# JohannesErnst/WeaSAL

Hardware: AMD Instinct MI355X
Metric: points/sec fwd+bwd KPFCNN on DALES spheres; achieved HBM GB/s on KPConv gather (higher is better)
Workload: dtype f32; 1 GPU; DALES_PseudoLabel KP-FCNN, in_radius=10m, 50k pts/sphere, batch=8, fp32, step = GPU pyramid + fwd + loss + bwd + SGD; contrast_loss term included (trainer_PseudoLabel.py:204-208); pyramid of the next batch overlapped on a second stream; parallelism=dp1, dist_world_size=1, allreduce_bytes=0

## Files before the change

### weasal_amd/_lib.py

```python
import ctypes as C
import os

_HERE = os.path.dirname(os.path.abspath(__file__))
LIB_PATH = os.path.join(_HERE, "libweasal_hip.so")

_vp = C.c_void_p
_i32 = C.c_int32
_i64 = C.c_int64
_f32 = C.c_float

SIGNATURES = {
    "ws_last_error": (C.c_char_p, []),
    "ws_version": (C.c_char_p, []),
    "ws_device_count": (C.c_int, []),
    "ws_kpconv_gather_fwd": (C.c_int, [_vp, _i64, _vp, _i64, _vp, _i32, _vp, _i32, _vp, _i32, _vp, _vp,
                                      _f32, _i32, _i32, _vp, _vp, _vp, _vp]),
    "ws_kpconv_gather_bwd_x": (C.c_int, [_vp, _i64, _vp, _i64, _vp, _i32, _vp, _vp, _vp, _i32, _vp, _i32,
                                        _vp, _vp, _f32, _i32, _i32, _vp, _vp, _vp]),
    "ws_kpconv_gather_bwd_geom": (C.c_int, [_vp, _i64, _vp, _i64, _vp, _i32, _vp, _i32, _vp, _vp, _i32,
                                           _vp, _vp, _vp, _f32, _i32, _i32, _vp, _vp, _vp]),
    "ws_transpose_scratch_bytes": (_i64, [_i64, _i32, _i64]),
    "ws_transpose_build": (C.c_int, [_vp, _i64, _i32, _i64, _vp, _vp, _vp, _vp]),
    "ws_max_pool_fwd": (C.c_int, [_vp, _i64, _i32, _vp, _i64, _i32, _vp, _vp, _vp]),
    "ws_max_pool_bwd": (C.c_int, [_vp, _vp, _i64, _i32, _i32, _vp, _vp, _i64, _vp, _vp]),
# ... 122 lines not shown
    "ws_region_mean_fwd": (C.c_int, [_vp, _i64, _i32, _vp, _vp, _i64, _vp, _i64, _vp, _vp]),
    "ws_region_mean_bwd": (C.c_int, [_vp, _i64, _i32, _vp, _vp, _i64, _vp, _i64, _vp, _vp]),
    "ws_sampler_create": (C.c_int, [C.POINTER(_vp)]),
    "ws_sampler_destroy": (None, [_vp]),
    "ws_sampler_add_cloud": (C.c_int, [_vp, _vp, _vp, _i64, _vp, _vp, _i64, _vp]),
    "ws_sampler_state_bytes": (_i64, []),
    "ws_sampler_draw_bytes": (_i64, []),
    "ws_sampler_batch": (C.c_int, [_vp, _vp, _i32, _i32, _i64, C.c_double, _f32, C.c_uint64, C.c_uint64, _i32, _vp, _i32, _i32, _i32,
                                   _vp, _vp, _vp, _vp, _vp, _vp, _vp, _vp, _vp, _i64, _vp, _vp]),
    "ws_softmax_ce_scratch_bytes": (_i64, [_i64]),
    "ws_softmax_ce_fwd": (C.c_int, [_vp, _i64, _i32, _i64, _vp, _vp, _i32, _vp, _vp, _vp, _vp, _vp]),
    "ws_softmax_ce_bwd": (C.c_int, [_vp, _i64, _i32, _i64, _vp, _vp, _i32, _vp, _vp, _vp, _vp, _i64, _vp]),
    "ws_sgd_step": (C.c_int, [_vp, _vp, _vp, _vp, _i32, _f32, _f32, _f32, _f32, _i32, _vp]),
    "ws_kpconv_deform_prepare": (C.c_int, [_vp, _i64, _i32, _vp, _i32, _f32, _i32, _vp, _vp, _vp, _vp, _vp]),
    "ws_kpconv_gather_fwd_ex": (C.c_int, [_vp, _i64, _vp, _i64, _vp, _i32, _vp, _i32, _vp, _i32, _vp, _vp, _f32, _i32, _i32, _vp,
                                         _vp, _vp, _i32, _i32, _vp]),
    "ws_kpconv_deform_prepare_bwd": (C.c_int, [_vp, _vp, _vp, _i64, _i32, _i32, _f32, _i32, _vp, _vp]),
    "ws_kpconv_gather_fwd_def": (C.c_int, [_vp, _i64, _vp, _i64, _vp, _i32, _vp, _i32, _vp, _i32, _f32, _vp, _vp, _vp, _i32, _i32, _vp]),
    "ws_kpconv_gather_bwd_x_def": (C.c_int, [_vp, _i64, _vp, _i64, _i32, _vp, _vp, _vp, _i32, _vp, _i32, _f32, _vp, _vp, _i32, _vp]),
    "ws_kpconv_gather_bwd_x_grid_wide": (C.c_int, [_vp, _i64, _vp, _i32, _i64, _vp, _f32, _vp, _i32, _vp, _i32, _vp, _vp, _f32, _vp,
                                                   _vp, _i32, _vp, _i32, _vp]),
    "ws_kpconv_gather_bwd_geom_def": (C.c_int, [_vp, _i64, _vp, _i64, _vp, _i32, _vp, _i32, _vp, _vp, _i32, _vp, _f32, _vp, _vp,
                                                _i32, _i32, _vp]),
    "ws_kpconv_layer_fwd_fused": (C.c_int, [_vp, _i64, _vp, _i64, _vp, _i32, _vp, _i32, _vp, _i32, _f32, _vp, _vp, _i32, _vp, _i32, _f32,
                                           _vp, _vp]),
    "ws_kpconv_gather_fwd_variant": (C.c_int, [_i32, _i32, _i32, _i32, _i32, _i32, C.c_char_p, _i32]),
    "ws_kpconv_gather_variant": (C.c_int, [_i32, _i64, _i64, _i32, _vp, _vp, _i32, _i32, _i32, _i32, _i32, _i32, _i32, C.c_char_p, _i32]),
    "ws_gemm_xb_variant": (C.c_int, [_vp, _i64, _i32, _i64, _vp, _i64, _i64, _i32, _vp, _vp, _i64, _vp, _i64, _vp, _i64, _vp, _i64,
                                     _vp, _i64, C.c_char_p, _i32]),
    "ws_gemm_xty_variant": (C.c_int, [_vp, _i64, _i32, _i64, _vp, _i32, _i64, _vp, _i64, _vp, _i32, C.c_char_p, _i32]),
    "ws_act_bwd_colsum_variant": (C.c_int, [_vp, _i64, _i32, _i64, _vp, _i64, _vp, _i64, _vp, _vp, C.c_char_p, _i32]),
    "ws_gemm_xbt_bf16_variant": (C.c_int, [_i64, _i32, _i32, _vp, _vp, _i64, _vp, _i64, _i32, C.c_char_p, _i32]),
    "ws_act_bwd_colsum_bf16_variant": (C.c_int, [_i32, _i64, _i32, _vp, _vp, C.c_char_p, _i32]),
    "ws_p2p_regularizer_scratch_bytes": (_i64, [_i64]),
    "ws_p2p_regularizer_fwd": (C.c_int, [_vp, _vp, _vp, _i64, _i32, _f32, _f32, _vp, _vp, _vp]),
    "ws_p2p_regularizer_bwd": (C.c_int, [_vp, _vp, _vp, _i64, _i32, _f32, _f32, _vp, _vp, _vp, _vp]),
    "ws_sphere_attention_fwd": (C.c_int, [_vp, _vp, _vp, _i64, _i32, _i32, _vp, _i32, _vp, _vp, _vp, _vp]),
    "ws_sphere_attention_bwd_scratch_bytes": (_i64, [_i64, _i32]),
    "ws_sphere_attention_bwd": (C.c_int, [_vp, _vp, _vp, _vp, _vp, _vp, _vp, _i64, _i32, _i32, _vp, _i32, _vp, _vp, _vp, _vp, _i64, _vp]),
    "ws_channel_attention_scratch_bytes": (_i64, [_vp, _i32, _i32, _i32]),
    "ws_channel_attention_fwd": (C.c_int, [_vp, _vp, _vp, _i64, _i32, _vp, _i32, _i32, _vp, _vp, _vp, _i64, _vp]),
    "ws_channel_attention_bwd": (C.c_int, [_vp, _vp, _vp, _vp, _vp, _i64, _i32, _vp, _i32, _i32, _vp, _vp, _vp, _vp, _i64, _vp]),
    "ws_timer_reset": (C.c_int, []),
    "ws_timer_count": (C.c_int, []),
    "ws_timer_read": (C.c_int, [_i32, _vp, _vp, _vp, _vp]),
    "ws_timer_read_layer": (C.c_int, [_i32, _vp]),
}

ENV_SWITCHES = (
    ("WEASAL_NB_WIDE_CAPS", "ws_nb_wide_caps"),
    ("WEASAL_CLOSEST_BWD_VEC", "ws_closest_bwd_vec"),
    ("WEASAL_GEMM_STAGED", "ws_gemm_staged"),
    ("WEASAL_GEMM_SHALLOW", "ws_gemm_shallow"),
)

_lib = None


class WeasalHipError(RuntimeError):
    pass


def lib():
    global _lib
    if _lib is None:
        if not os.path.exists(LIB_PATH):
            raise WeasalHipError(
                "%s not found: build it with `python -c 'import __graft_entry__ as g; g.build()'` "
                "or `make -C weasal_amd/csrc` (there is no CPU fallback)" % LIB_PATH)
        handle = C.CDLL(LIB_PATH)
        for name, (res, args) in SIGNATURES.items():
            fn = getattr(handle, name)
            fn.restype = res
            fn.argtypes = args
        for env, sym in ENV_SWITCHES:
            if env in os.environ:
                C.c_int.in_dll(handle, sym).value = int(os.environ[env])
        _lib = handle
    return _lib


def check(rc):
    if rc != 0:
        msg = lib().ws_last_error()
        raise WeasalHipError("libweasal_hip status %d: %s" % (rc, msg.decode() if msg else "?"))


def ptr(t):
    return None if t is None else _vp(t.data_ptr())


_raw_stream = None


def current_stream():
    global _raw_stream
    import torch
    if _raw_stream is None:
        get = getattr(torch._C, "_cuda_getCurrentRawStream", None)
        dev = getattr(torch._C, "_cuda_getDevice", None)
        if get is not None and dev is not None and torch.cuda.is_available():
            torch.cuda.current_stream()
            _raw_stream = lambda: get(dev())
        else:
            _raw_stream = lambda: torch.cuda.current_stream().cuda_stream
    return _vp(_raw_stream())
# ... 1 lines not shown
```

### weasal_amd/csrc/kpconv.hip

```cpp
#include "ws_common.h"
#include <algorithm>
#include "ws_grid.h"
#include "ws_bf16.h"

namespace {

constexpr float WS_SHADOW = 1e6f;

struct GeomParams {
    float extent;
    int influence;
    int aggregation;
    int deformable;
    const void* gate;
    float gate_slope;
    const int64_t* rows;
    int rows_h;
    const float4* kp4;
    const float* rmax;
    int cut;
    int ilv;
    int csplit;
};

template <int K>
__device__ __forceinline__ void kp_influence(float nx, float ny, float nz, const float* __restrict__ kp,
                                             const GeomParams& g, bool live, float (&w)[K], float (&d2)[K])
{
    float best = 3.4e38f;
    int arg = 0;
    bool inrange = false;
    const float e2 = g.extent * g.extent;
#pragma unroll
    for (int k = 0; k < K; ++k) {
        const float dx = nx - kp[3 * k + 0];
        const float dy = ny - kp[3 * k + 1];
        const float dz = nz - kp[3 * k + 2];
        const float d = (dx * dx + dy * dy) + dz * dz;
        d2[k] = d;
        if (d < best) { best = d; arg = k; }
        inrange |= d < e2;
    }
#pragma unroll
    for (int k = 0; k < K; ++k) {
        float v;
        if (g.influence == WS_INFLUENCE_LINEAR) {
            v = fmaxf(1.0f - sqrtf(d2[k]) / g.extent, 0.0f);
        } else if (g.influence == WS_INFLUENCE_CONSTANT) {
            v = 1.0f;
        } else {
            const float sig = g.extent * 0.3f;
            v = expf(-d2[k] / (2.0f * sig * sig + 1e-9f));
        }
        if (g.aggregation == WS_AGGREGATION_CLOSEST && k != arg) v = 0.0f;
// ... 1407 lines not shown
            }
        }
#pragma unroll
        for (int r = 0; r < 4; ++r) {
#pragma unroll
            for (int o = 1; o < 16; o <<= 1) {
                gk[r][0] += __shfl_xor(gk[r][0], o, 64);
                gk[r][1] += __shfl_xor(gk[r][1], o, 64);
                gk[r][2] += __shfl_xor(gk[r][2], o, 64);
                gm[r] += __shfl_xor(gm[r], o, 64);
                const float ob = __shfl_xor(best[r], o, 64);
                const int oc = __shfl_xor(bestcol[r], o, 64);
                const bool take = ob < best[r] || (ob == best[r] && oc < bestcol[r]);
                best[r] = take ? ob : best[r];
                bestcol[r] = take ? oc : bestcol[r];
            }
            const int k = 4 * g + r;
            if (k < K) {
                float gx = gk[r][0], gy = gk[r][1], gz = gk[r][2];
                if (d_min_d2) {
                    const int64_t v = inds[q * h + min(bestcol[r], h - 1)];
                    float mx = WS_SHADOW, my = WS_SHADOW, mz = WS_SHADOW;
                    if (v >= 0 && v < ns) { mx = s_pts[3 * v]; my = s_pts[3 * v + 1]; mz = s_pts[3 * v + 2]; }
                    const float gmin = 2.0f * d_min_d2[q * K + k];
                    gx = fmaf(gmin, kq[r].x - (mx - qx), gx);
                    gy = fmaf(gmin, kq[r].y - (my - qy), gy);
                    gz = fmaf(gmin, kq[r].z - (mz - qz), gz);
                }
                if (j == 0) d_kp4[q * K + k] = make_float4(gx, gy, gz, gm[r]);
            }
        }
    }
}

bool aligned16(const void* p) { return (reinterpret_cast<uintptr_t>(p) & 15u) == 0; }

int check_common(const void* q_pts, int64_t nq, const void* s_pts, int64_t ns, int32_t h, int32_t ci,
                 int32_t k, float extent, int32_t influence, int32_t aggregation)
{
    WS_REQUIRE(nq >= 0 && ns >= 0, "negative point count (nq=%lld ns=%lld)", (long long)nq, (long long)ns);
    WS_REQUIRE(h >= 1 && ci >= 1, "h=%d and ci=%d must be >= 1", h, ci);
    WS_REQUIRE(nq == 0 || q_pts, "q_pts is NULL");
    WS_REQUIRE(ns == 0 || s_pts, "s_pts is NULL");
    WS_REQUIRE(extent > 0.0f, "KP_extent must be > 0");
    WS_REQUIRE(influence >= 0 && influence <= 2, "unknown influence %d", influence);
    WS_REQUIRE(aggregation >= 0 && aggregation <= 1, "unknown aggregation %d", aggregation);
    WS_REQUIRE(ns < (1ll << 31) && nq * (int64_t)k < (1ll << 31), "index range exceeds int32");
    if (k != 15) return ws_fail(WS_ERR_UNSUPPORTED, "num_kernel_points=%d: this build instantiates K=15 only", k);
    return WS_OK;
}

constexpr int GRID_SLAB = 192;

template <int K, int G, int MODE, bool VEC, typename T = float, bool SORT = true>
__global__ __launch_bounds__(256) void kpconv_gather_bwd_x_grid_kernel(
    const float* __restrict__ s_pts, int64_t ns, const CloudGrid* __restrict__ grids, int nb,
    const int32_t* __restrict__ cell_start, const float4* __restrict__ sorted,
    const unsigned long long* __restrict__ key_last, float r2, const T* __restrict__ dwf, int ci,
    const float* __restrict__ kernel_points, const float* __restrict__ deformed_kp, const float* __restrict__ modulations,
    GeomParams g, T* __restrict__ dx, const int32_t* __restrict__ order, int32_t* __restrict__ overflow)
{
    constexpr int CC = 4 * G;
    constexpr int S = 64 / G;
    constexpr int EPL = GRID_SLAB / 64;
    __shared__ uint2 pool_all[4][POOL_ALLOC];
    __shared__ int segs_all[4][K + 1];
    __shared__ float4 slab_all[4][GRID_SLAB + 64];
    const int wave = __builtin_amdgcn_readfirstlane(threadIdx.x >> 6);
    const int lane = threadIdx.x & 63;
    uint2* pool = pool_all[wave];
    int* segs = segs_all[wave];
    float4* slab = slab_all[wave];
    const int j = lane % G;
    const int slot = lane / G;
    const float inv_extent = 1.0f / g.extent;

    float kpr[MODE == 0 ? 3 * K : 1];
    if (MODE == 0) {
#pragma unroll
        for (int t = 0; t < 3 * K; ++t) kpr[t] = kernel_points[t];
    }

    int64_t item0, istep, iend;
    ws_wave_items(ns, order ? g.ilv : 0, wave, item0, istep, iend);
    CloudGrid gr = grids[0];
    for (int64_t item = item0; item < iend; item += istep) {
        const int64_t s = order ? (int64_t)order[item] : item;
        if (s < gr.s_base || s >= gr.s_base + gr.s_len) {
            int b = 0;
            while (b + 1 < nb && s >= grids[b].s_base + grids[b].s_len) ++b;
            gr = grids[b];
        }
        const float sx = s_pts[3 * s + 0], sy = s_pts[3 * s + 1], sz = s_pts[3 * s + 2];
        int cnt = 0;
        auto take = [&](const float4& c, bool active) {
            const float d2 = ref_d2(c.x, c.y, c.z, make_float4(sx, sy, sz, 0.0f));
            const unsigned long long key = ((unsigned long long)__float_as_uint(d2) << 32) | (unsigned)s;
            bool hit = active && d2 < r2;
            hit = hit && key <= key_last[hit ? __float_as_int(c.w) : 0];
            const unsigned long long m = __ballot(hit);
            const int pos = cnt + lane_rank(m);
            slab[(hit && pos < GRID_SLAB) ? pos : GRID_SLAB + lane] = c;
            cnt += __builtin_popcountll(m);
        };
        const bool from_row = g.rows != nullptr && key_last[s] == ~0ull;
        if (from_row) {
            for (int h0 = 0; h0 < g.rows_h; h0 += 64) {
                const int col = h0 + lane;
                const int64_t qi = col < g.rows_h ? g.rows[s * g.rows_h + col] : -1;
                const bool active = qi >= 0 && qi < ns;
                const int64_t qq = active ? qi : 0;
                take(make_float4(s_pts[3 * qq + 0], s_pts[3 * qq + 1], s_pts[3 * qq + 2], __int_as_float((int)qq)), active);
            }
        } else if (gr.s_len > 0) {
            const int cx = cell_coord(sx, gr.lo[0], gr.inv_cell);
            const int cy = cell_coord(sy, gr.lo[1], gr.inv_cell);
            const int cz = cell_coord(sz, gr.lo[2], gr.inv_cell);
            const int x0 = max(cx - 1, 0), x1 = min(cx + 1, gr.nx - 1);
            int rb[9], re[9];
#pragma unroll
            for (int r = 0; r < 9; ++r) {
                const int z = cz + r / 3 - 1, y = cy + r % 3 - 1;
                const bool ok = x0 <= x1 && z >= 0 && z < gr.nz && y >= 0 && y < gr.ny;
                const int row = gr.cell_base + ((ok ? z : 0) * gr.ny + (ok ? y : 0)) * gr.nx;
                rb[r] = ok ? cell_start[row + x0] : 0;
                re[r] = ok ? cell_start[row + x1 + 1] : 0;
            }
            float4 c[9];
#pragma unroll
            for (int r = 0; r < 9; ++r) {
                const int p = rb[r] + lane;
                c[r] = sorted[p < re[r] ? p : 0];
            }
#pragma unroll
            for (int r = 0; r < 9; ++r) {
                take(c[r], rb[r] + lane < re[r]);
                for (int p0 = rb[r] + 64; p0 < re[r]; p0 += 64) {
                    const int p = p0 + lane;
                    float4 cc = make_float4(0.f, 0.f, 0.f, 0.f);
                    if (p < re[r]) cc = sorted[p];
                    take(cc, p < re[r]);
                }
            }
        }
        if (cnt > GRID_SLAB) {
            if (lane == 0) atomicMax(overflow, cnt);
            cnt = GRID_SLAB;
        }
        wave_lds_sync();
        if (SORT) {
            float4 e[EPL];
            int rk[EPL];
#pragma unroll
            for (int u = 0; u < EPL; ++u) {
                e[u] = lane + 64 * u < cnt ? slab[lane + 64 * u] : make_float4(0.f, 0.f, 0.f, __int_as_float(0x7fffffff));
                rk[u] = 0;
            }
            if (cnt <= 64) {
                for (int i = 0; i < cnt; ++i) rk[0] += __float_as_int(slab[i].w) < __float_as_int(e[0].w) ? 1 : 0;
            } else if (cnt <= 128) {
                for (int i = 0; i < cnt; ++i) {
                    const int ki = __float_as_int(slab[i].w);
                    rk[0] += ki < __float_as_int(e[0].w) ? 1 : 0;
                    rk[1] += ki < __float_as_int(e[1].w) ? 1 : 0;
                }
            } else {
                for (int i = 0; i < cnt; ++i) {
                    const int ki = __float_as_int(slab[i].w);
#pragma unroll
                    for (int u = 0; u < EPL; ++u) rk[u] += ki < __float_as_int(e[u].w) ? 1 : 0;
                }
            }
            wave_lds_sync();
#pragma unroll
            for (int u = 0; u < EPL; ++u)
                if (lane + 64 * u < cnt) slab[rk[u]] = e[u];
            wave_lds_sync();
        }
        for (int cc0 = 0; cc0 < ci; cc0 += CC) {
            float4 acc = make_float4(0.f, 0.f, 0.f, 0.f);
            const int ch = cc0 + 4 * j;
            const bool chok = VEC ? (ch + 3 < ci) : (ch < ci);
            const int chl = chok ? ch : 0;
            float4 gq = make_float4(1.f, 1.f, 1.f, 1.f);
            if (g.gate && slot == 0) {
                const T* gy = reinterpret_cast<const T*>(g.gate) + s * ci + ch;
                if (VEC) {
                    if (chok) gq = ld4(gy);
                } else {
                    if (ch + 0 < ci) gq.x = ld1(gy + 0);
                    if (ch + 1 < ci) gq.y = ld1(gy + 1);
                    if (ch + 2 < ci) gq.z = ld1(gy + 2);
                    if (ch + 3 < ci) gq.w = ld1(gy + 3);
                }
            }
            auto flush = [&](int total) {
                wave_lds_sync();
                total = min(total, POOL);
                const int per = (total + S - 1) / S;
                const int lo = slot * per;
                const int hi = chok ? min(lo + per, total) : lo;
                for (int it = 0; it < per; it += 4) {
                    float4 v[4];
                    float w[4];
                    uint2 e[4];
#pragma unroll
                    for (int u = 0; u < 4; ++u) {
                        e[u] = pool[min(lo + it + u, POOL + 7)];
                        keep_unconditional(e[u]);
                    }
#pragma unroll
                    for (int u = 0; u < 4; ++u) {
                        const bool ok = lo + it + u < hi;
                        e[u].x = ok ? e[u].x : 0u;
                        w[u] = ok ? __uint_as_float(e[u].y) : 0.0f;
                        v[u] = load_row_piece<VEC>(dwf, e[u].x, ci, chl);
                    }
#pragma unroll
                    for (int u = 0; u < 4; ++u) {
                        acc.x = fmaf(w[u], v[u].x, acc.x);
                        acc.y = fmaf(w[u], v[u].y, acc.y);
                        acc.z = fmaf(w[u], v[u].z, acc.z);
                        acc.w = fmaf(w[u], v[u].w, acc.w);
                    }
                }
                wave_lds_sync();
            };
            for (int p0 = 0; p0 < cnt; p0 += 64) {
                const int p = p0 + lane;
                const bool real = p < cnt;
                const float4 c = real ? slab[p] : make_float4(0.f, 0.f, 0.f, 0.f);
                const int q = real ? __float_as_int(c.w) : 0;
                const float nx = sx - c.x, ny = sy - c.y, nz = sz - c.z;
                const float* lkp = deformed_kp ? deformed_kp + (int64_t)q * (3 * K) : kernel_points;
                const float* lmod = modulations ? modulations + (int64_t)q * K : nullptr;
                auto kp = [&](int k, int cidx) { return MODE == 0 ? kpr[MODE == 0 ? 3 * k + cidx : 0] : lkp[3 * k + cidx]; };
                auto nomin = [&](int, float) {};
                int total = 0, maxlen = 0;
                kp_list<K, MODE>(nx, ny, nz, real, kp, g, inv_extent, (unsigned)(q * K), 1u, lmod, pool, segs, lane, total,
                                 maxlen, nomin);
                if (total <= POOL) {
                    flush(total);
                } else {
                    for (int sub = 0; sub < 4; ++sub) {
                        total = 0; maxlen = 0;
                        kp_list<K, MODE>(nx, ny, nz, real && (lane >> 4) == sub, kp, g, inv_extent, (unsigned)(q * K), 1u, lmod,
                                         pool, segs, lane, total, maxlen, nomin);
                        flush(total);
                    }
                }
            }
#pragma unroll
            for (int o = G; o < 64; o <<= 1) {
                acc.x += __shfl_xor(acc.x, o, 64);
                acc.y += __shfl_xor(acc.y, o, 64);
                acc.z += __shfl_xor(acc.z, o, 64);
                acc.w += __shfl_xor(acc.w, o, 64);
            }
            if (slot == 0) {
                T* dst = dx + s * ci + ch;
                if (g.gate) {
                    acc.x *= gq.x > 0.0f ? 1.0f : g.gate_slope; acc.y *= gq.y > 0.0f ? 1.0f : g.gate_slope;
                    acc.z *= gq.z > 0.0f ? 1.0f : g.gate_slope; acc.w *= gq.w > 0.0f ? 1.0f : g.gate_slope;
                }
                if (VEC) {
                    if (chok) st4(dst, acc);
                } else {
                    if (ch + 0 < ci) st1(dst + 0, acc.x);
                    if (ch + 1 < ci) st1(dst + 1, acc.y);
                    if (ch + 2 < ci) st1(dst + 2, acc.z);
                    if (ch + 3 < ci) st1(dst + 3, acc.w);
                }
            }
        }
        wave_lds_sync();
    }
}


template <int K, int G, int MODE, bool VEC, int NCH, typename T = float>
__global__ __launch_bounds__(256) void kpconv_gather_bwd_x_gridw_kernel(
    const float* __restrict__ s_pts, int64_t ns, const CloudGrid* __restrict__ grids, int nb,
    const int32_t* __restrict__ cell_start, const float4* __restrict__ sorted,
    const unsigned long long* __restrict__ key_last, float r2, const T* __restrict__ dwf, int ci,
    const float* __restrict__ kernel_points, const float* __restrict__ deformed_kp, const float* __restrict__ modulations,
    GeomParams g, T* __restrict__ dx, const int32_t* __restrict__ order)
{
    constexpr int CC = 4 * G;
    constexpr int S = 64 / G;
    static_assert(NCH == 1 || NCH == 2 || NCH == 4, "channel chunks whose accumulators stay in registers");
    constexpr int SLAB = 192;
    __shared__ uint2 pool_all[4][POOL_ALLOC];
    __shared__ int segs_all[4][K + 1];
    __shared__ float4 slab_all[4][SLAB + 64];
    __shared__ int2 runs_all[4][16];
    const int wave = __builtin_amdgcn_readfirstlane(threadIdx.x >> 6);
    const int lane = threadIdx.x & 63;
    uint2* pool = pool_all[wave];
    int* segs = segs_all[wave];
    float4* slab = slab_all[wave];
    int2* runs = runs_all[wave];
    const int j = lane % G;
    const int slot = lane / G;
    const float inv_extent = 1.0f / g.extent;

    float kpr[MODE == 0 ? 3 * K : 1];
    float cut2 = 3.4e38f;
    if (MODE == 0) {
#pragma unroll
        for (int t = 0; t < 3 * K; ++t) kpr[t] = kernel_points[t];
        float rr = 0.0f;
#pragma unroll
        for (int k = 0; k < K; ++k) rr = fmaxf(rr, (kpr[3 * k] * kpr[3 * k] + kpr[3 * k + 1] * kpr[3 * k + 1]) + kpr[3 * k + 2] * kpr[3 * k + 2]);
        const float R = (__builtin_sqrtf(rr) + g.extent) * 1.0001f;
        cut2 = R * R;
    } else if (MODE == 2 && g.rmax) {
        const float R = (g.rmax[0] + g.extent) * 1.0001f;
        cut2 = R * R;
    }

    int64_t item0, istep, iend;
    ws_wave_items(ns, order ? g.ilv : 0, wave, item0, istep, iend);
    CloudGrid gr = grids[0];
    for (int64_t item = item0; item < iend; item += istep) {
        const int64_t s = order ? (int64_t)order[item] : item;
        if (s < gr.s_base || s >= gr.s_base + gr.s_len) {
            int b = 0;
            while (b + 1 < nb && s >= grids[b].s_base + grids[b].s_len) ++b;
// ... 177 lines not shown
                    auto kp = [&](int k, int cidx) { return MODE == 0 ? kpr[MODE == 0 ? 3 * k + cidx : 0] : lkp[3 * k + cidx]; };
                    auto nomin = [&](int, float) {};
                    kp_list<K, MODE == 2 ? 1 : MODE>(nx, ny, nz, real, kp, g, inv_extent, (unsigned)(q * K), 1u, lmod, pool, segs, lane,
                                                     total, maxlen, nomin);
                    if (total <= POOL) {
                        flush(total);
                    } else {
                        for (int sub = 0; sub < 4; ++sub) {
                            total = 0; maxlen = 0;
                            kp_list<K, MODE == 2 ? 1 : MODE>(nx, ny, nz, real && (lane >> 4) == sub, kp, g, inv_extent, (unsigned)(q * K),
                                                             1u, lmod, pool, segs, lane, total, maxlen, nomin);
                            flush(total);
                        }
                    }
                }
            }
#pragma unroll
            for (int c = 0; c < NCH; ++c) {
                if (cg0 + c * CC >= ci) continue;
#pragma unroll
                for (int o = G; o < 64; o <<= 1) {
                    acc[c].x += __shfl_xor(acc[c].x, o, 64);
                    acc[c].y += __shfl_xor(acc[c].y, o, 64);
                    acc[c].z += __shfl_xor(acc[c].z, o, 64);
                    acc[c].w += __shfl_xor(acc[c].w, o, 64);
                }
                if (slot == 0) {
                    const int ch = cg0 + c * CC + 4 * j;
                    T* dst = dx + s * ci + ch;
                    float4 a = acc[c];
                    if (g.gate) {
                        a.x *= gq[c].x > 0.0f ? 1.0f : g.gate_slope; a.y *= gq[c].y > 0.0f ? 1.0f : g.gate_slope;
                        a.z *= gq[c].z > 0.0f ? 1.0f : g.gate_slope; a.w *= gq[c].w > 0.0f ? 1.0f : g.gate_slope;
                    }
                    if (VEC) {
                        if (chok[c]) st4(dst, a);
                    } else {
                        if (ch + 0 < ci) st1(dst + 0, a.x);
                        if (ch + 1 < ci) st1(dst + 1, a.y);
                        if (ch + 2 < ci) st1(dst + 2, a.z);
                        if (ch + 3 < ci) st1(dst + 3, a.w);
                    }
                }
            }
            wave_lds_order();
        }
    }
}

}

extern "C" int ws_kpconv_grid_sorted;
int ws_kpconv_grid_sorted = 0;

#include <cstdio>
#include <type_traits>

namespace {

constexpr int SPLIT_ROWS = 4096;
constexpr int PACK_MEAN_MAX = 12;
constexpr int SPLIT_NT = 4;
constexpr int GRID_INTERLEAVE = 512;

enum { GK_FWD_MFMA, GK_FWD_POOL, GK_BWD_X, GK_BWD_GEOM, GK_BWD_X_GRID, GK_BWD_X_GRIDW, GK_BWD_GEOM_DEF, GK_BWD_X_PACKED };
struct GatherPlan {
    int kernel;
    bool bf16;
    int n;
    int mode;
    bool def;
    bool vec;
    int pw;
    bool cut;
    int nch;
    bool sort;
    bool areg;
    int grid;
    int csplit, ilv, rows_sorted;
};

int nt_for_rows(int ci, const void* a, const void* b)
{
    const int nt = ci <= 16 ? 1 : (ci <= 32 ? 2 : (ci <= 64 ? 4 : (ci <= 128 ? 8 : 16)));
    return (ci % nt == 0 && (nt == 1 || (aligned16(a) && aligned16(b)))) ? nt : 1;
}
int group_ladder(int ci) { return ci <= 4 ? 1 : (ci <= 8 ? 2 : (ci <= 16 ? 4 : (ci <= 32 ? 8 : 16))); }
bool rows_vec4(bool bf16, int ci, const void* a, const void* b)
{
    return ci % 4 == 0 && (bf16 ? ws_row_aligned<bf16_t>(a) && ws_row_aligned<bf16_t>(b) : ws_row_aligned<float>(a) && ws_row_aligned<float>(b));
}
int rows_vec4_or_f32(bool bf16, int ci, const void* a, const void* b, bool& vec4)
{
    vec4 = rows_vec4(bf16, ci, a, b);
    WS_REQUIRE(!bf16 || vec4, "bf16 feature rows need ci %% 4 == 0 and 8-byte aligned rows (ci=%d)", ci);
    return WS_OK;
}
bool rigid_fast(bool deformed, bool modulated, int influence, int aggregation)
{
    return !deformed && !modulated && influence == WS_INFLUENCE_LINEAR && aggregation == WS_AGGREGATION_SUM;
}
void grid_walk_plan(int64_t ns, bool ordered, GatherPlan& p)
{
    p.ilv = ordered ? GRID_INTERLEAVE : 0;
    p.grid = p.ilv > 0 ? 8 * (int)std::max<int64_t>(1, std::min<int64_t>(p.ilv, ws_ceil_div(ns, 32))) : ws_grid(ns, 4);
}

GatherPlan new_plan(int kernel, bool bf16, int64_t items)
{
    GatherPlan p{};
    p.kernel = kernel; p.bf16 = bf16; p.csplit = 1; p.grid = ws_grid(items, 4);
    return p;
}

int fwd_plan(bool bf16, int64_t nq, int32_t ci, const void* x, const void* wf, bool deformed, bool modulated, int32_t influence,
             int32_t aggregation, bool rows_sorted, GatherPlan& p)
{
    p = new_plan(ci > 4 ? GK_FWD_MFMA : GK_FWD_POOL, bf16, nq);
    p.def = deformed; p.rows_sorted = rows_sorted;
    if (int rc = rows_vec4_or_f32(bf16, ci, x, wf, p.vec)) return rc;
    if (ci > 4) {
        const bool fastm = rigid_fast(deformed, modulated, influence, aggregation);
        p.n = nt_for_rows(ci, x, wf);
        p.mode = fastm ? 0 : 1; p.vec = true; p.cut = fastm && rows_sorted;
        if (fastm && !rows_sorted && nq < SPLIT_ROWS) {
            if (p.n > SPLIT_NT && ci % SPLIT_NT == 0) p.n = SPLIT_NT;
            if (ci > 16 * p.n) {
                p.csplit = (ci + 16 * p.n - 1) / (16 * p.n);
                p.grid = ws_grid(nq * p.csplit, 4);
            }
        }
        return WS_OK;
    }
    p.mode = (!deformed && influence == WS_INFLUENCE_LINEAR && aggregation == WS_AGGREGATION_SUM) ? 0 : 1;
    p.n = p.vec ? 1 : 4; p.pw = p.vec ? 4 : 1;
    return WS_OK;
}

int fwd_def_plan(bool bf16, int64_t nq, int32_t ci, const void* x, const void* wf, bool rows_sorted, GatherPlan& p)
{
    p = new_plan(GK_FWD_MFMA, bf16, nq);
    p.n = nt_for_rows(ci, x, wf);
    p.mode = 2; p.def = true; p.vec = true; p.cut = rows_sorted;
    if (bf16 && p.n == 1 && (ci % 2)) return ws_fail(WS_ERR_UNSUPPORTED, "bf16 rows need an even channel count (ci=%d)", ci);
    return WS_OK;
}

int bwd_x_plan(bool bf16, int64_t ns, int32_t ci, const void* dwf, const void* dx, int mode, GatherPlan& p)
{
    p = new_plan(GK_BWD_X, bf16, ns);
    p.n = group_ladder(ci); p.mode = mode;
    return rows_vec4_or_f32(bf16, ci, dwf, dx, p.vec);
}

int bwd_x_packed_plan(bool bf16, int64_t nq, int64_t ns, int32_t h, int32_t ci, const void* dwf, const void* dx, int mode, bool ordered,
                      GatherPlan& p)
{
    if (int rc = bwd_x_plan(bf16, ns, ci, dwf, dx, mode, p)) return rc;
    (void)ordered;
    if (bf16 || !p.vec || mode != 0 || nq >= ns || nq * (int64_t)h > (int64_t)PACK_MEAN_MAX * ns) return WS_OK;
    p.kernel = GK_BWD_X_PACKED;
    p.grid = ws_grid(ws_ceil_div(ns, 4), 4);
    return WS_OK;
}

int bwd_geom_plan(bool bf16, int64_t nq, int32_t ci, const void* x, const void* dwf, GatherPlan& p)
{
    p = new_plan(GK_BWD_GEOM, bf16, nq);
    p.mode = 1; p.vec = rows_vec4(bf16, ci, x, dwf);
    return WS_OK;
}

int bwd_x_grid_plan(bool bf16, int64_t ns, int32_t ci, const void* dwf, const void* dx, int mode, bool ordered, GatherPlan& p)
{
    p = new_plan(GK_BWD_X_GRID, bf16, ns);
    p.n = group_ladder(ci); p.mode = mode; p.sort = ws_kpconv_grid_sorted != 0;
    grid_walk_plan(ns, ordered, p);
    return rows_vec4_or_f32(bf16, ci, dwf, dx, p.vec);
}

int bwd_x_gridw_plan(bool bf16, int64_t ns, int32_t ci, const void* dwf, const void* dx, bool deformed, bool ordered, GatherPlan& p)
{
    p = new_plan(GK_BWD_X_GRIDW, bf16, ns);
    p.n = group_ladder(ci); p.mode = deformed ? 2 : 0;
    p.nch = (p.n < 16 || ci <= 64) ? 1 : (ci <= 128 ? 2 : 4);
    grid_walk_plan(ns, ordered, p);
    return rows_vec4_or_f32(bf16, ci, dwf, dx, p.vec);
}

int bwd_geom_def_plan(bool bf16, int64_t nq, int32_t ci, const void* x, const void* dwf, bool rows_sorted, GatherPlan& p)
{
    p = new_plan(GK_BWD_GEOM_DEF, bf16, nq);
    if (ci % 16 != 0 || !aligned16(x) || !aligned16(dwf))
        return ws_fail(WS_ERR_UNSUPPORTED, "geometry backward on the matrix core needs ci %% 16 == 0 and 16-byte aligned rows (ci=%d)", ci);
    p.mode = 2; p.vec = true; p.cut = rows_sorted;
    p.areg = ci == 16 || ci == 32 || ci == 64 || ci == 128;
    p.n = p.areg ? ci / 4 : (ci % 128 == 0 ? 32 : (ci % 64 == 0 ? 16 : (ci % 32 == 0 ? 8 : 4)));
    return WS_OK;
}

void plan_text(const GatherPlan& p, char* out, size_t n)
{
    const char* t = p.bf16 ? "bf16" : "float";
    auto b = [](bool v) { return v ? "true" : "false"; };
    switch (p.kernel) {
    case GK_FWD_MFMA:
        snprintf(out, n, "kpconv_gather_fwd_mfma_kernel<NT=%d, MODE=%d, DEF=%s, VECROW=%s, T=%s, CUT=%s> grid=%d csplit=%d", p.n, p.mode,
                 b(p.def), b(p.vec), t, b(p.cut), p.grid, p.csplit);
        break;
    case GK_FWD_POOL:
        snprintf(out, n, "kpconv_gather_fwd_kernel<K=15, G=%d, MODE=%d, DEF=%s, VEC=%s, PW=%d, T=%s> grid=%d csplit=%d cut=%d", p.n, p.mode,
                 b(p.def), b(p.vec), p.pw, t, p.grid, p.csplit, p.rows_sorted);
        break;
    case GK_BWD_X:
        snprintf(out, n, "kpconv_gather_bwd_x_kernel<K=15, G=%d, MODE=%d, VEC=%s, T=%s> grid=%d", p.n, p.mode, b(p.vec), t, p.grid);
        break;
    case GK_BWD_X_PACKED:
        snprintf(out, n, "kpconv_gather_bwd_x_packed_kernel<K=15, G=%d, VEC=%s, T=%s> grid=%d", p.n, b(p.vec), t, p.grid);
        break;
    case GK_BWD_GEOM:
        snprintf(out, n, "kpconv_gather_bwd_geom_kernel<K=15, T=%s> grid=%d vec4=%d", t, p.grid, p.vec ? 1 : 0);
        break;
    case GK_BWD_X_GRID:
        snprintf(out, n, "kpconv_gather_bwd_x_grid_kernel<K=15, G=%d, MODE=%d, VEC=%s, T=%s, SORT=%s> grid=%d ilv=%d", p.n, p.mode, b(p.vec),
                 t, b(p.sort), p.grid, p.ilv);
        break;
    case GK_BWD_X_GRIDW:
        snprintf(out, n, "kpconv_gather_bwd_x_gridw_kernel<K=15, G=%d, MODE=%d, VEC=%s, NCH=%d, T=%s> grid=%d ilv=%d", p.n, p.mode,
                 b(p.vec), p.nch, t, p.grid, p.ilv);
        break;
    default:
        snprintf(out, n, "kpconv_gather_bwd_geom_def_kernel<CK=%d, AREG=%s, T=%s, CUT=%s> grid=%d", p.n, b(p.areg), t, b(p.cut), p.grid);
    }
}

template <int... Vs> struct Pick { int v; };
using Flag = Pick<0, 1>;
template <typename F> void dispatch(F&& f) { f(); }
template <typename F, int... Vs, typename... Rest>
void dispatch(F&& f, Pick<Vs...> a, Rest... rest)
{
    (void)(((a.v == Vs) && (dispatch([&](auto... cs) { f(std::integral_constant<int, Vs>{}, cs...); }, rest...), true)) || ...);
}
template <int BF> using Row = std::conditional_t<BF != 0, bf16_t, float>;
int launched() { WS_LAUNCH_CHECK(); return WS_OK; }

__global__ __launch_bounds__(256) void kp4_rmax_kernel(const float4* __restrict__ kp4, int64_t n, int* __restrict__ rmax_bits)
{
#pragma clang fp contract(off)
    int64_t e = (int64_t)blockIdx.x * 256 + threadIdx.x;
    if (e >= n) e = n - 1;
    const float4 v = kp4[e];
    float r = sqrtf((v.x * v.x + v.y * v.y) + v.z * v.z);
#pragma unroll
    for (int o = 32; o > 0; o >>= 1) r = fmaxf(r, __shfl_xor(r, o, 64));
    if ((threadIdx.x & 63) == 0 && __float_as_int(r) > *(volatile int*)rmax_bits) atomicMax(rmax_bits, __float_as_int(r));
}

struct GridView {
    const CloudGrid* grids;
    const int32_t* cell_start;
    const float4* sorted;
    const unsigned long long* key_last;
    float r2;
};
GridView grid_view(const void* grid_blob, int32_t nb, int64_t cells, const uint64_t* key_last, float radius)
{
    const char* base = (const char*)grid_blob;
    return GridView{(const CloudGrid*)base, (const int32_t*)(base + ws_grid_blob_cells_off(nb)),
                    (const float4*)(base + ws_grid_blob_sorted_off(nb, cells)), reinterpret_cast<const unsigned long long*>(key_last),
                    radius * radius};
}

void launch_fwd_mfma(const GatherPlan& p, void* stream, const float* q_pts, int64_t nq, const float* s_pts, int64_t ns, const int64_t* inds,
                     int32_t h, const void* x, int32_t ci, const float* kernel_points, const float* deformed_kp, const float* modulations,
                     const GeomParams& g, void* wf, float* min_d2, const int32_t* order)
{
    dispatch([&](auto bf, auto nt, auto mode, auto def, auto cut) {
// ... 36 lines not shown
    WS_REQUIRE(t_offsets && t_pairs && dwf && dx && (kernel_points || deformed_kp), "NULL argument");
    WS_REQUIRE(nq * (int64_t)h < (1ll << 31), "nq*h exceeds int32");
    WS_REQUIRE(nq * (int64_t)k * ci < (1ll << 31), "nq*k*ci exceeds the 32-bit row offsets of the gather");
    GatherPlan p;
    const int mode = rigid_fast(deformed_kp, modulations, influence, aggregation) ? 0 : 1;
    if (int rc = packed ? bwd_x_packed_plan(bf16, nq, ns, h, ci, dwf, dx, mode, order != nullptr, p) : bwd_x_plan(bf16, ns, ci, dwf, dx, mode, p))
        return rc;
    GeomParams g{extent, influence, aggregation, deformed_kp ? 1 : 0, gate, gate_slope, nullptr, 0};
    if (p.kernel == GK_BWD_X_PACKED) {
        launch_bwd_x_packed(p, stream, q_pts, nq, s_pts, ns, h, t_offsets, t_pairs, (const float*)dwf, ci, kernel_points, g, (float*)dx, order);
        return launched();
    }
    launch_bwd_x(p, stream, q_pts, nq, s_pts, ns, h, t_offsets, t_pairs, dwf, ci, kernel_points, deformed_kp, modulations, g, dx, order);
    return launched();
}

int gather_bwd_geom_impl(bool bf16, const float* q_pts, int64_t nq, const float* s_pts, int64_t ns, const int64_t* inds, int32_t h,
                         const void* x, int32_t ci, const void* dwf, int32_t k, const float* deformed_kp, const float* modulations,
                         const float* d_min_d2, float extent, int32_t influence, int32_t aggregation, float* d_deformed_kp,
                         float* d_modulations, void* stream)
{
    if (int rc = check_common(q_pts, nq, s_pts, ns, h, ci, k, extent, influence, aggregation)) return rc;
    if (nq == 0) return WS_OK;
    WS_REQUIRE(inds && x && dwf && deformed_kp && d_deformed_kp, "NULL argument");
    GatherPlan p;
    if (int rc = bwd_geom_plan(bf16, nq, ci, x, dwf, p)) return rc;
    GeomParams g{extent, influence, aggregation, 1, nullptr, 0.0f, nullptr, 0};
    dispatch([&](auto bf) {
        using T = Row<bf.value>;
        kpconv_gather_bwd_geom_kernel<15, T><<<p.grid, 256, 0, (hipStream_t)stream>>>(
            q_pts, nq, s_pts, ns, inds, h, (const T*)x, ci, (const T*)dwf, deformed_kp, modulations, d_min_d2, g, d_deformed_kp, d_modulations,
            p.vec);
    }, Flag{p.bf16});
    return launched();
}

int gather_bwd_x_grid_impl(bool bf16, const float* s_pts, int64_t ns, const void* grid_blob, int32_t nb, int64_t cells,
                           const uint64_t* key_last, float radius, const void* dwf, int32_t ci, const float* kernel_points, int32_t k,
                           const float* deformed_kp, const float* modulations, float extent, int32_t influence, int32_t aggregation,
                           const int32_t* order, void* dx, int32_t* overflow, void* stream, const void* gate = nullptr,
                           float gate_slope = 0.0f, const int64_t* rows = nullptr, int32_t rows_h = 0)
{
    if (int rc = check_common(s_pts, ns, s_pts, ns, 1, ci, k, extent, influence, aggregation)) return rc;
    if (ns == 0) return WS_OK;
    WS_REQUIRE(grid_blob && key_last && dwf && dx && overflow && (kernel_points || deformed_kp), "NULL argument");
    WS_REQUIRE(nb >= 1 && cells >= 1, "bad grid nb=%d cells=%lld", nb, (long long)cells);
    WS_REQUIRE(ns * (int64_t)k * ci < (1ll << 31), "ns*k*ci exceeds the 32-bit row offsets of the gather");
    WS_REQUIRE(!rows || rows_h >= 1, "index rows given without their width");
    GatherPlan p;
    const int mode = rigid_fast(deformed_kp, modulations, influence, aggregation) ? 0 : 1;
    if (int rc = bwd_x_grid_plan(bf16, ns, ci, dwf, dx, mode, order != nullptr, p)) return rc;
    GeomParams g{extent, influence, aggregation, deformed_kp ? 1 : 0, gate, gate_slope, rows, rows_h, nullptr, nullptr, 0, p.ilv};
    const GridView v = grid_view(grid_blob, nb, cells, key_last, radius);
    dispatch([&](auto bf, auto gr, auto md, auto vec, auto sort) {
        using T = Row<bf.value>;
        if constexpr (!bf.value || vec.value)
            kpconv_gather_bwd_x_grid_kernel<15, gr.value, md.value, vec.value != 0, T, sort.value != 0><<<p.grid, 256, 0, (hipStream_t)stream>>>(
                s_pts, ns, v.grids, nb, v.cell_start, v.sorted, v.key_last, v.r2, (const T*)dwf, ci, kernel_points, deformed_kp, modulations, g,
                (T*)dx, order, overflow);
    }, Flag{p.bf16}, Pick<1, 2, 4, 8, 16>{p.n}, Pick<0, 1>{p.mode}, Flag{p.vec}, Flag{p.sort});
    return launched();
}

}

extern "C" {

int ws_kpconv_gather_fwd_ex(const float* q_pts, int64_t nq, const float* s_pts, int64_t ns, const int64_t* inds, int32_t h,
                            const void* x, int32_t ci, const float* kernel_points, int32_t k, const float* deformed_kp,
                            const float* modulations, float extent, int32_t influence, int32_t aggregation, const int32_t* order,
                            void* wf, float* min_d2, int32_t rows_bf16, int32_t rows_sorted, void* stream)
{
    if (int rc = check_common(q_pts, nq, s_pts, ns, h, ci, k, extent, influence, aggregation)) return rc;
    if (nq == 0) return WS_OK;
    WS_REQUIRE(inds && x && wf && (kernel_points || deformed_kp), "NULL argument");
    WS_REQUIRE(ns * (int64_t)ci < (1ll << 31), "ns*ci exceeds the 32-bit row offsets of the gather");
    GatherPlan p;
    if (int rc = fwd_plan(rows_bf16 != 0, nq, ci, x, wf, deformed_kp, modulations, influence, aggregation, rows_sorted != 0, p)) return rc;
    GeomParams g{extent, influence, aggregation, deformed_kp ? 1 : 0, nullptr, 0.0f, nullptr, 0, nullptr, nullptr, p.rows_sorted, 0, p.csplit};
    if (p.kernel == GK_FWD_MFMA)
        launch_fwd_mfma(p, stream, q_pts, nq, s_pts, ns, inds, h, x, ci, kernel_points, deformed_kp, modulations, g, wf, min_d2, order);
    else
        dispatch([&](auto bf, auto vec, auto mode, auto def) {
            using T = Row<bf.value>;
            if constexpr ((!bf.value || vec.value) && (mode.value == 1 || !def.value))
                kpconv_gather_fwd_kernel<15, vec.value ? 1 : 4, mode.value, def.value != 0, vec.value != 0, vec.value ? 4 : 1, T>
                    <<<p.grid, 256, 0, (hipStream_t)stream>>>(
                    q_pts, nq, s_pts, ns, inds, h, (const T*)x, ci, kernel_points, deformed_kp, modulations, g, (T*)wf, min_d2, order);
        }, Flag{p.bf16}, Flag{p.vec}, Pick<0, 1>{p.mode}, Flag{p.def});
    return launched();
}

int ws_kpconv_gather_fwd(const float* q_pts, int64_t nq, const float* s_pts, int64_t ns,
                         const int64_t* inds, int32_t h, const float* x, int32_t ci,
                         const float* kernel_points, int32_t k, const float* deformed_kp,
                         const float* modulations, float extent, int32_t influence, int32_t aggregation,
                         const int32_t* order, float* wf, float* min_d2, void* stream)
{
    return ws_kpconv_gather_fwd_ex(q_pts, nq, s_pts, ns, inds, h, x, ci, kernel_points, k, deformed_kp, modulations, extent, influence,
                                   aggregation, order, wf, min_d2, 0, 0, stream);
}

int ws_kpconv_gather_fwd_bf16(const float* q_pts, int64_t nq, const float* s_pts, int64_t ns,
                              const int64_t* inds, int32_t h, const uint16_t* x, int32_t ci,
                              const float* kernel_points, int32_t k, const float* deformed_kp,
                              const float* modulations, float extent, int32_t influence, int32_t aggregation,
                              const int32_t* order, uint16_t* wf, float* min_d2, void* stream)
{
    return ws_kpconv_gather_fwd_ex(q_pts, nq, s_pts, ns, inds, h, x, ci, kernel_points, k, deformed_kp, modulations, extent, influence,
                                   aggregation, order, wf, min_d2, 1, 0, stream);
}

int ws_kpconv_gather_fwd_def(const float* q_pts, int64_t nq, const float* s_pts, int64_t ns, const int64_t* inds, int32_t h,
// ... 271 lines not shown
```

Baseline: 32.67 million points/s.

## Software-pipeline per-item loads in KPConv grid backward-x kernel

Adds a PIPE variant of the grid backward-x gather kernel that prefetches the item index, point coordinates, key_last and the first row of neighbour indices up to three items ahead. Each item's global-load latency is meant to hide behind the current item's accumulation work. The variant also swaps full wave LDS syncs for a lighter ordering barrier and narrows the loop counter to 32 bits. It is enabled by default for vectorised rows and raises register pressure, which could lower occupancy.

```diff
diff --git a/weasal_amd/_lib.py b/weasal_amd/_lib.py
--- a/weasal_amd/_lib.py
+++ b/weasal_amd/_lib.py
@@ -198,6 +198,7 @@
     ("WEASAL_CLOSEST_BWD_VEC", "ws_closest_bwd_vec"),
     ("WEASAL_GEMM_STAGED", "ws_gemm_staged"),
     ("WEASAL_GEMM_SHALLOW", "ws_gemm_shallow"),
+    ("WEASAL_GRID_PIPELINE", "ws_kpconv_grid_pipeline"),
 )
 
 _lib = None
diff --git a/weasal_amd/csrc/kpconv.hip b/weasal_amd/csrc/kpconv.hip
--- a/weasal_amd/csrc/kpconv.hip
+++ b/weasal_amd/csrc/kpconv.hip
@@ -1,5 +1,6 @@
 #include "ws_common.h"
 #include <algorithm>
+#include <type_traits>
 #include "ws_grid.h"
 #include "ws_bf16.h"
 
@@ -1513,7 +1514,7 @@
 
 constexpr int GRID_SLAB = 192;
 
-template <int K, int G, int MODE, bool VEC, typename T = float, bool SORT = true>
+template <int K, int G, int MODE, bool VEC, typename T = float, bool SORT = true, bool PIPE = false>
 __global__ __launch_bounds__(256) void kpconv_gather_bwd_x_grid_kernel(
     const float* __restrict__ s_pts, int64_t ns, const CloudGrid* __restrict__ grids, int nb,
     const int32_t* __restrict__ cell_start, const float4* __restrict__ sorted,
@@ -1535,6 +1536,10 @@
     const int j = lane % G;
     const int slot = lane / G;
     const float inv_extent = 1.0f / g.extent;
+    auto lds_sync = [&]() {
+        if constexpr (PIPE) wave_lds_order();
+        else wave_lds_sync();
+    };
 
     float kpr[MODE == 0 ? 3 * K : 1];
     if (MODE == 0) {
@@ -1545,62 +1550,136 @@
     int64_t item0, istep, iend;
     ws_wave_items(ns, order ? g.ilv : 0, wave, item0, istep, iend);
     CloudGrid gr = grids[0];
-    for (int64_t item = item0; item < iend; item += istep) {
-        const int64_t s = order ? (int64_t)order[item] : item;
-        if (s < gr.s_base || s >= gr.s_base + gr.s_len) {
-            int b = 0;
-            while (b + 1 < nb && s >= grids[b].s_base + grids[b].s_len) ++b;
-            gr = grids[b];
-        }
-        const float sx = s_pts[3 * s + 0], sy = s_pts[3 * s + 1], sz = s_pts[3 * s + 2];
+    int a_s = -1, b_s = -1, c_s = -1, b_qq = -1, c_qq = -1, gb = 0;
+    bool b_from = false, c_from = false;
+    float b_px = 0.f, b_py = 0.f, b_pz = 0.f, c_px = 0.f, c_py = 0.f, c_pz = 0.f, c_cx = 0.f, c_cy = 0.f, c_cz = 0.f;
+    unsigned long long c_kq = 0ull;
+    int vz = 0;
+    if constexpr (PIPE) asm volatile("" : "+v"(vz));
+    auto uniform_i = [](int v) { return __builtin_amdgcn_readfirstlane(v); };
+    auto uniform_f = [](float v) { return __builtin_bit_cast(float, __builtin_amdgcn_readfirstlane(__builtin_bit_cast(int, v))); };
+    using Item = std::conditional_t<PIPE, int, int64_t>;
+    const Item wstep = (Item)istep, wend = (Item)iend;
+    for (Item item = PIPE ? (Item)item0 - 3 * wstep : (Item)item0; item < wend; item += wstep) {
+        int n_s = -1;
+        float n_px = 0.f, n_py = 0.f, n_pz = 0.f, n_cx = 0.f, n_cy = 0.f, n_cz = 0.f;
+        unsigned long long n_kl = 0ull, n_kq = 0ull;
+        int64_t n_row = -1;
+        auto prefetch = [&]() {
+            const int i3 = (int)item + 3 * (int)wstep;
+            if (i3 < (int)wend) n_s = order ? order[i3 + vz] : i3 + vz;
+            {
+                const int64_t sa = (a_s >= 0 ? a_s : 0) + vz;
+                n_px = s_pts[3 * sa + 0]; n_py = s_pts[3 * sa + 1]; n_pz = s_pts[3 * sa + 2];
+                n_kl = key_last[sa];
+                if (g.rows) n_row = g.rows[sa * g.rows_h + min(lane, g.rows_h - 1)];
+            }
+            if (b_from) {
+                const int64_t qs = b_qq >= 0 ? b_qq : 0;
+                n_cx = s_pts[3 * qs + 0]; n_cy = s_pts[3 * qs + 1]; n_cz = s_pts[3 * qs + 2];
+                n_kq = key_last[qs];
+            }
+        };
+        auto rotate = [&]() {
+            c_s = b_s; c_px = uniform_f(b_px); c_py = uniform_f(b_py); c_pz = uniform_f(b_pz); c_from = b_from;
+            c_qq = b_qq; c_cx = n_cx; c_cy = n_cy; c_cz = n_cz; c_kq = n_kq;
+            b_s = a_s; b_px = n_px; b_py = n_py; b_pz = n_pz;
+            b_from = g.rows != nullptr && b_s >= 0 && uniform_i((int)(n_kl == ~0ull)) != 0;
+            b_qq = (lane < g.rows_h && n_row >= 0 && n_row < ns) ? (int)n_row : -1;
+            a_s = uniform_i(n_s);
+        };
+        if (PIPE && c_s < 0) {
+            prefetch();
+            rotate();
+            continue;
+        }
+        int64_t s;
+        float sx, sy, sz;
+        if constexpr (PIPE) {
+            s = c_s;
+            sx = c_px; sy = c_py; sz = c_pz;
+        } else {
+            s = order ? (int64_t)order[item] : item;
+            if (s < gr.s_base || s >= gr.s_base + gr.s_len) {
+                int b = 0;
+                while (b + 1 < nb && s >= grids[b].s_base + grids[b].s_len) ++b;
+                gr = grids[b];
+            }
+            sx = s_pts[3 * s + 0]; sy = s_pts[3 * s + 1]; sz = s_pts[3 * s + 2];
+        }
         int cnt = 0;
-        auto take = [&](const float4& c, bool active) {
+        auto near = [&](const float4& c, bool active, unsigned long long& key) {
             const float d2 = ref_d2(c.x, c.y, c.z, make_float4(sx, sy, sz, 0.0f));
-            const unsigned long long key = ((unsigned long long)__float_as_uint(d2) << 32) | (unsigned)s;
-            bool hit = active && d2 < r2;
-            hit = hit && key <= key_last[hit ? __float_as_int(c.w) : 0];
+            key = ((unsigned long long)__float_as_uint(d2) << 32) | (unsigned)s;
+            return active && d2 < r2;
+        };
+        auto put = [&](const float4& c, bool hit) {
             const unsigned long long m = __ballot(hit);
             const int pos = cnt + lane_rank(m);
             slab[(hit && pos < GRID_SLAB) ? pos : GRID_SLAB + lane] = c;
             cnt += __builtin_popcountll(m);
         };
-        const bool from_row = g.rows != nullptr && key_last[s] == ~0ull;
+        auto take = [&](const float4& c, bool active) {
+            unsigned long long key;
+            bool hit = near(c, active, key);
+            hit = hit && key <= key_last[hit ? __float_as_int(c.w) : 0];
+            put(c, hit);
+        };
+        const bool from_row = PIPE ? c_from : (g.rows != nullptr && key_last[s] == ~0ull);
         if (from_row) {
-            for (int h0 = 0; h0 < g.rows_h; h0 += 64) {
+            if constexpr (PIPE) {
+                const bool active = c_qq >= 0;
+                const float4 c = make_float4(c_cx, c_cy, c_cz, __int_as_float(active ? c_qq : 0));
+                unsigned long long key;
+                bool hit = near(c, active, key);
+                hit = hit && key <= c_kq;
+                put(c, hit);
+            }
+            for (int h0 = PIPE ? 64 : 0; h0 < g.rows_h; h0 += 64) {
                 const int col = h0 + lane;
                 const int64_t qi = col < g.rows_h ? g.rows[s * g.rows_h + col] : -1;
                 const bool active = qi >= 0 && qi < ns;
                 const int64_t qq = active ? qi : 0;
                 take(make_float4(s_pts[3 * qq + 0], s_pts[3 * qq + 1], s_pts[3 * qq + 2], __int_as_float((int)qq)), active);
             }
-        } else if (gr.s_len > 0) {
-            const int cx = cell_coord(sx, gr.lo[0], gr.inv_cell);
-            const int cy = cell_coord(sy, gr.lo[1], gr.inv_cell);
-            const int cz = cell_coord(sz, gr.lo[2], gr.inv_cell);
-            const int x0 = max(cx - 1, 0), x1 = min(cx + 1, gr.nx - 1);
-            int rb[9], re[9];
-#pragma unroll
-            for (int r = 0; r < 9; ++r) {
-                const int z = cz + r / 3 - 1, y = cy + r % 3 - 1;
-                const bool ok = x0 <= x1 && z >= 0 && z < gr.nz && y >= 0 && y < gr.ny;
-                const int row = gr.cell_base + ((ok ? z : 0) * gr.ny + (ok ? y : 0)) * gr.nx;
-                rb[r] = ok ? cell_start[row + x0] : 0;
-                re[r] = ok ? cell_start[row + x1 + 1] : 0;
-            }
-            float4 c[9];
-#pragma unroll
-            for (int r = 0; r < 9; ++r) {
-                const int p = rb[r] + lane;
-                c[r] = sorted[p < re[r] ? p : 0];
-            }
-#pragma unroll
-            for (int r = 0; r < 9; ++r) {
-                take(c[r], rb[r] + lane < re[r]);
-                for (int p0 = rb[r] + 64; p0 < re[r]; p0 += 64) {
-                    const int p = p0 + lane;
-                    float4 cc = make_float4(0.f, 0.f, 0.f, 0.f);
-                    if (p < re[r]) cc = sorted[p];
-                    take(cc, p < re[r]);
+        } else {
+            if constexpr (PIPE) {
+                gr = grids[gb];
+                if (s < gr.s_base || s >= gr.s_base + gr.s_len) {
+                    gb = 0;
+                    while (gb + 1 < nb && s >= grids[gb].s_base + grids[gb].s_len) ++gb;
+                    gr = grids[gb];
+                }
+            }
+            if (gr.s_len > 0) {
+                const int cx = cell_coord(sx, gr.lo[0], gr.inv_cell);
+                const int cy = cell_coord(sy, gr.lo[1], gr.inv_cell);
+                const int cz = cell_coord(sz, gr.lo[2], gr.inv_cell);
+                const int x0 = max(cx - 1, 0), x1 = min(cx + 1, gr.nx - 1);
+                int rb[9], re[9];
+#pragma unroll
+                for (int r = 0; r < 9; ++r) {
+                    const int z = cz + r / 3 - 1, y = cy + r % 3 - 1;
+                    const bool ok = x0 <= x1 && z >= 0 && z < gr.nz && y >= 0 && y < gr.ny;
+                    const int row = gr.cell_base + ((ok ? z : 0) * gr.ny + (ok ? y : 0)) * gr.nx;
+                    rb[r] = ok ? cell_start[row + x0] : 0;
+                    re[r] = ok ? cell_start[row + x1 + 1] : 0;
+                }
+                float4 c[9];
+#pragma unroll
+                for (int r = 0; r < 9; ++r) {
+                    const int p = rb[r] + lane;
+                    c[r] = sorted[p < re[r] ? p : 0];
+                }
+#pragma unroll
+                for (int r = 0; r < 9; ++r) {
+                    take(c[r], rb[r] + lane < re[r]);
+                    for (int p0 = rb[r] + 64; p0 < re[r]; p0 += 64) {
+                        const int p = p0 + lane;
+                        float4 cc = make_float4(0.f, 0.f, 0.f, 0.f);
+                        if (p < re[r]) cc = sorted[p];
+                        take(cc, p < re[r]);
+                    }
                 }
             }
         }
@@ -1608,7 +1687,8 @@
             if (lane == 0) atomicMax(overflow, cnt);
             cnt = GRID_SLAB;
         }
-        wave_lds_sync();
+        if constexpr (PIPE) prefetch();
+        lds_sync();
         if (SORT) {
             float4 e[EPL];
             int rk[EPL];
@@ -1632,11 +1712,11 @@
                     for (int u = 0; u < EPL; ++u) rk[u] += ki < __float_as_int(e[u].w) ? 1 : 0;
                 }
             }
-            wave_lds_sync();
+            lds_sync();
 #pragma unroll
             for (int u = 0; u < EPL; ++u)
                 if (lane + 64 * u < cnt) slab[rk[u]] = e[u];
-            wave_lds_sync();
+            lds_sync();
         }
         for (int cc0 = 0; cc0 < ci; cc0 += CC) {
             float4 acc = make_float4(0.f, 0.f, 0.f, 0.f);
@@ -1656,7 +1736,7 @@
                 }
             }
             auto flush = [&](int total) {
-                wave_lds_sync();
+                lds_sync();
                 total = min(total, POOL);
                 const int per = (total + S - 1) / S;
                 const int lo = slot * per;
@@ -1685,7 +1765,7 @@
                         acc.w = fmaf(w[u], v[u].w, acc.w);
                     }
                 }
-                wave_lds_sync();
+                lds_sync();
             };
             for (int p0 = 0; p0 < cnt; p0 += 64) {
                 const int p = p0 + lane;
@@ -1721,6 +1801,7 @@
             if (slot == 0) {
                 T* dst = dx + s * ci + ch;
                 if (g.gate) {
+                    if constexpr (PIPE) asm volatile("" : "+v"(gq.x), "+v"(gq.y), "+v"(gq.z), "+v"(gq.w));
                     acc.x *= gq.x > 0.0f ? 1.0f : g.gate_slope; acc.y *= gq.y > 0.0f ? 1.0f : g.gate_slope;
                     acc.z *= gq.z > 0.0f ? 1.0f : g.gate_slope; acc.w *= gq.w > 0.0f ? 1.0f : g.gate_slope;
                 }
@@ -1734,7 +1815,8 @@
                 }
             }
         }
-        wave_lds_sync();
+        lds_sync();
+        if constexpr (PIPE) rotate();
     }
 }
 
@@ -2018,6 +2100,8 @@
 
 extern "C" int ws_kpconv_grid_sorted;
 int ws_kpconv_grid_sorted = 0;
+extern "C" int ws_kpconv_grid_pipeline;
+int ws_kpconv_grid_pipeline = 1;
 
 #include <cstdio>
 #include <type_traits>
@@ -2041,6 +2125,7 @@
     bool cut;
     int nch;
     bool sort;
+    bool pipe;
     bool areg;
     int grid;
     int csplit, ilv, rows_sorted;
@@ -2140,9 +2225,10 @@
 int bwd_x_grid_plan(bool bf16, int64_t ns, int32_t ci, const void* dwf, const void* dx, int mode, bool ordered, GatherPlan& p)
 {
     p = new_plan(GK_BWD_X_GRID, bf16, ns);
-    p.n = group_ladder(ci); p.mode = mode; p.sort = ws_kpconv_grid_sorted != 0;
-    grid_walk_plan(ns, ordered, p);
-    return rows_vec4_or_f32(bf16, ci, dwf, dx, p.vec);
+    p.n = group_ladder(ci); p.mode = mode; p.sort = ws_kpconv_grid_sorted != 0; grid_walk_plan(ns, ordered, p);
+    if (int rc = rows_vec4_or_f32(bf16, ci, dwf, dx, p.vec)) return rc;
+    p.pipe = ws_kpconv_grid_pipeline != 0 && p.vec;
+    return WS_OK;
 }
 
 int bwd_x_gridw_plan(bool bf16, int64_t ns, int32_t ci, const void* dwf, const void* dx, bool deformed, bool ordered, GatherPlan& p)
@@ -2188,8 +2274,8 @@
         snprintf(out, n, "kpconv_gather_bwd_geom_kernel<K=15, T=%s> grid=%d vec4=%d", t, p.grid, p.vec ? 1 : 0);
         break;
     case GK_BWD_X_GRID:
-        snprintf(out, n, "kpconv_gather_bwd_x_grid_kernel<K=15, G=%d, MODE=%d, VEC=%s, T=%s, SORT=%s> grid=%d ilv=%d", p.n, p.mode, b(p.vec),
-                 t, b(p.sort), p.grid, p.ilv);
+        snprintf(out, n, "kpconv_gather_bwd_x_grid_kernel<K=15, G=%d, MODE=%d, VEC=%s, T=%s, SORT=%s> grid=%d ilv=%d pipe=%d", p.n, p.mode,
+                 b(p.vec), t, b(p.sort), p.grid, p.ilv, p.pipe ? 1 : 0);
         break;
     case GK_BWD_X_GRIDW:
         snprintf(out, n, "kpconv_gather_bwd_x_gridw_kernel<K=15, G=%d, MODE=%d, VEC=%s, NCH=%d, T=%s> grid=%d ilv=%d", p.n, p.mode,
@@ -2332,13 +2418,14 @@
     if (int rc = bwd_x_grid_plan(bf16, ns, ci, dwf, dx, mode, order != nullptr, p)) return rc;
     GeomParams g{extent, influence, aggregation, deformed_kp ? 1 : 0, gate, gate_slope, rows, rows_h, nullptr, nullptr, 0, p.ilv};
     const GridView v = grid_view(grid_blob, nb, cells, key_last, radius);
-    dispatch([&](auto bf, auto gr, auto md, auto vec, auto sort) {
+    dispatch([&](auto bf, auto gr, auto md, auto vec, auto sort, auto pipe) {
         using T = Row<bf.value>;
-        if constexpr (!bf.value || vec.value)
-            kpconv_gather_bwd_x_grid_kernel<15, gr.value, md.value, vec.value != 0, T, sort.value != 0><<<p.grid, 256, 0, (hipStream_t)stream>>>(
+        if constexpr ((!bf.value || vec.value) && (!pipe.value || vec.value))
+            kpconv_gather_bwd_x_grid_kernel<15, gr.value, md.value, vec.value != 0, T, sort.value != 0, pipe.value != 0>
+                <<<p.grid, 256, 0, (hipStream_t)stream>>>(
                 s_pts, ns, v.grids, nb, v.cell_start, v.sorted, v.key_last, v.r2, (const T*)dwf, ci, kernel_points, deformed_kp, modulations, g,
                 (T*)dx, order, overflow);
-    }, Flag{p.bf16}, Pick<1, 2, 4, 8, 16>{p.n}, Pick<0, 1>{p.mode}, Flag{p.vec}, Flag{p.sort});
+    }, Flag{p.bf16}, Pick<1, 2, 4, 8, 16>{p.n}, Pick<0, 1>{p.mode}, Flag{p.vec}, Flag{p.sort}, Flag{p.pipe});
     return launched();
 }
 
```

After: 32.65 million points/s. No clear change (-0.1%).
